# irap-omp/deconv3d

Hardware: AMD Instinct MI355X
Metric: spaxel-updates/sec (MH-Gibbs) (higher is better)
Workload: dtype f64; 1 GPU; c3_300x300x128; fsf=moffat 11x11, lsf_taps=17, spaxels=90000, lsf=analytic MUSE stand-in (mpdaf absent), parallelism=1 chain, variance=per-voxel cube (heteroscedastic)

## Files before the change

deconv3d_amd/csrc/d3d_api.hip:

```cpp
#include "d3d_ctx.h"

#include <dlfcn.h>

#define D3D_VERSION 300
#ifndef D3D_SOURCE_HASH
#define D3D_SOURCE_HASH "unknown"
#endif

namespace {
thread_local std::string g_err;
}

namespace d3dh {
int fail(int code, const char *fmt, ...) {
    char buf[512];
    va_list ap;
    va_start(ap, fmt);
    vsnprintf(buf, sizeof buf, fmt, ap);
    va_end(ap);
    g_err = buf;
    return code;
}
}

// ... 89 lines not shown
    c->mh_nt_ivar = c->mh_nt_ivar && fits_raw;
    c->mh_layers_forced = c->mh_layers_opt > 0;
    c->mh_layers_cfg = c->mh_layers_forced ? c->mh_layers_opt : 2;
    if (c->mh_layers_cfg < 1) c->mh_layers_cfg = 1;
    if (c->mh_layers_cfg > d3d::MH_LAYERS) c->mh_layers_cfg = d3d::MH_LAYERS;
    if (c->Dp > 160 && c->mh_layers_cfg > 2) c->mh_layers_cfg = 2;
    c->mh_defer = c->mh_defer_opt;
    c->mh_zb = c->mh_zblocks && c->Dp > d3d::MH_WS_MAX_DP && c->mh_defer == 1 && !c->mh_flow &&
               (!c->have_taps || c->ntaps == 0 || c->lsf_dense_any);
    if (c->mh_defer != 1 || c->mh_flow || (c->Dp > d3d::MH_WS_MAX_DP && !c->mh_zb)) c->mh_layers_cfg = 1;
    if (c->deep && !c->mh_zb) c->mh_defer = 0;
    c->mh_layers = c->mh_layers_cfg;
}

int floor_div(int a, int b) { return a >= 0 ? a / b : -((-a + b - 1) / b); }

int build_colour_lists(d3d_ctx *c) {
    const int ncol = c->fh * c->fw;
    const int fhh = (c->fh - 1) / 2, fhw = (c->fw - 1) / 2;
    c->parts.clear();
    if (c->part_rects.empty()) {
        d3d_ctx::Part pt;
        pt.y0 = c->oy0;
        pt.y1 = c->oy1;
        pt.x0 = c->ox0;
        pt.x1 = c->ox1;
        c->parts.push_back(pt);
        c->n_phases = 1;
    } else {
        c->n_phases = 1;
// ... 45 lines not shown
                    }
                if (pt.real[col] > 0) {
                    const long n_all_col =
                        ((long)list.size() - pt.off[col]) * (c->mh_zb ? (c->Dp + 255) / 256 : 1);
                    if (c->mh_zigzag && (ord & 1) && n_all_col > c->flow_grid) {
                        std::reverse(list.begin() + pt.off[col], list.begin() + pt.off[col] + pt.real[col]);
                        std::reverse(list.begin() + pt.off[col] + pt.real[col], list.end());
                    }
                    ++ord;
                }
                most = std::max(most, (int)list.size() - pt.off[col]);
            }
        pt.off[ncol] = (int)list.size();
        const long most_wgs = (long)most * (c->mh_zb ? (c->Dp + 255) / 256 : 1);
        pt.layers = (!c->mh_layers_forced && most_wgs < c->flow_grid / 2) ? 1 : c->mh_layers_cfg;
        const bool partitioned = c->tiled || !c->part_rects.empty();
        pt.wide = pt.layers == 1 && c->mh_wide && partitioned && c->Dp == 128 && most > 0 &&
                  most <= c->flow_grid / 4 && c->mh_defer == 1;
        pt.small = pt.layers == 1 && most_wgs < c->flow_grid / 2;
        pt.chain = false;
        pt.K = 0;
        pt.last_col = -1;
        for (int col = 0; col < ncol; ++col)
            if (pt.real[col] > 0) {
                ++pt.K;
                pt.last_col = col;
            }
#ifdef D3D_EXPERIMENTS
        if (!empty && pt.K > 0) {
            const int cus = c->flow_grid / 4;
// ... 50 lines not shown
                HIP_TRY(hipMemsetAsync(c->chain_flags, 0, 2 * need_slots * sizeof(unsigned), c->stream));
                c->chain_base = 0;
            }
            if (need_G > c->chain_G_cap) {
                if (c->chain_G) (void)hipFree(c->chain_G);
                c->chain_G = nullptr;
                c->chain_G_cap = 0;
                HIP_TRY(hipMalloc(&c->chain_G, need_G * sizeof(double)));
                c->chain_G_cap = need_G;
            }
            HIP_TRY(hipStreamSynchronize(c->stream));
        }
    }
    c->mh_layers = 1;
    for (const d3d_ctx::Part &pt : c->parts) c->mh_layers = std::max(c->mh_layers, pt.layers);
    if (list.size() > c->spx_cap) {
        if (c->spx) (void)hipFree(c->spx);
        c->spx = nullptr;
        c->spx_cap = 0;
        HIP_TRY(hipMalloc(&c->spx, list.size() * sizeof(int4)));
        c->spx_cap = list.size();
    }
    c->flow_K = 0;
    c->flow_items = 0;
    c->flow_last_cy = c->flow_last_cx = -1;
#ifdef D3D_EXPERIMENTS
    if (!c->tiled && c->parts.size() == 1 && list.size() <= c->flow_cap_items) {
        const d3d_ctx::Part &pt = c->parts[0];
        std::vector<int4> ents, cols;
        std::vector<int> lat((size_t)ncol * c->flow_LY * c->flow_LX, -1);
// ... 314 lines not shown
    CTX_TRY(hipMalloc(&c->dlog, (size_t)c->HW * sizeof(double)));
    CTX_TRY(hipMalloc(&c->hwbuf, (size_t)c->HW * sizeof(double)));
    CTX_TRY(hipMalloc(&c->scal, 16 * sizeof(double)));
    CTX_TRY(hipMalloc(&c->accepted, sizeof(unsigned long long)));
    CTX_TRY(hipMalloc(&c->acc_map, (size_t)c->HW * sizeof(unsigned)));
    c->spx_cap = (size_t)(H + 2 * fh) * (W + 2 * fw);
    CTX_TRY(hipMalloc(&c->spx, c->spx_cap * sizeof(int4)));
    c->slots_x = (W + fw - 1) / fw;
    c->slots = c->slots_x * ((H + fh - 1) / fh);
    c->Wg = W;
    c->oy1 = H;
    c->ox1 = W;
    CTX_TRY(hipMalloc(&c->prev, (size_t)c->HW * 3 * sizeof(double)));
    CTX_TRY(hipMalloc(&c->recbuf, (size_t)c->HW * 8 * sizeof(double)));
    CTX_TRY(hipMalloc(&c->idxbuf, (size_t)c->HW * sizeof(int)));
    for (int b = 0; b < 4; ++b) {
        CTX_TRY(hipMalloc(&c->gbuf[b], (size_t)c->slots * c->Dp * sizeof(double)));
        CTX_TRY(hipMemsetAsync(c->gbuf[b], 0, (size_t)c->slots * c->Dp * sizeof(double), c->stream));
    }
    {
#ifdef D3D_EXPERIMENTS
        const size_t ncol = (size_t)fh * fw;
        c->flow_LY = H / fh + 3;
        c->flow_LX = W / fw + 3;
        c->flow_cap_K = ncol;
        c->flow_cap_items = c->spx_cap;
        CTX_TRY(hipMalloc(&c->flow_ent, c->spx_cap * sizeof(int4)));
        CTX_TRY(hipMalloc(&c->flow_col, ncol * sizeof(int4)));
        CTX_TRY(hipMalloc(&c->flow_lat, ncol * c->flow_LY * c->flow_LX * sizeof(int)));
        c->flow_state_bytes = ((4 + ncol + c->spx_cap) * sizeof(unsigned) + 15) / 16 * 16;
        CTX_TRY(hipMalloc(&c->flow_state, c->flow_state_bytes));
// ... 32 lines not shown
    }
    if (c->copy_stream) (void)hipStreamDestroy(c->copy_stream);
    if (c->halo_send) (void)hipFree(c->halo_send);
    if (c->halo_recv) (void)hipFree(c->halo_recv);
    for (double *p : c->post_cube)
        if (p) (void)hipFree(p);
    if (c->post_map) (void)hipFree(c->post_map);
    hist_free(c);
    adapt_free(c);
    if (c->prior_part) (void)hipFree(c->prior_part);
    for (hipEvent_t e : c->halo_ev) (void)hipEventDestroy(e);
    for (int s = 0; s < D3D_SLOT_COUNT; ++s)
        if (c->slot[s]) (void)hipFree(c->slot[s]);
    if (c->line.tab) (void)hipFree(const_cast<double *>(c->line.tab));
    void *ptrs[] = {c->stage, c->stage2, c->params, c->params_alt, c->mask, c->fsf, c->lsf_shift, c->lsf_weight,
                    c->dlog, c->hwbuf, c->scal, c->accepted, c->acc_map, c->spx, c->gbuf[0], c->gbuf[1], c->gbuf[2], c->gbuf[3],
                    c->flow_ent, c->flow_col, c->flow_lat, c->flow_state, c->flow_err, c->pair_state, c->sep_uv,
                    c->lsf_dense, c->prev, c->recbuf, c->idxbuf, c->extbuf, c->fsf_quad, c->fsf_quad_sep,
                    c->chain_cols, c->chain_flags, c->chain_G, c->props, c->z_part, c->z_E, c->ltab, c->ptab};
    for (void *p : ptrs)
        if (p) (void)hipFree(p);
#ifdef D3D_EXPERIMENTS
    if (c->stampbuf) (void)hipFree(c->stampbuf);
#endif
    if (c->ev0) (void)hipEventDestroy(c->ev0);
    if (c->ev1) (void)hipEventDestroy(c->ev1);
    if (c->own_stream) (void)hipStreamDestroy(c->own_stream);
    delete c;
    return D3D_OK;
}

// ... 73 lines not shown
        long n = 0;
        for (const d3d_ctx::Part &pt : c->parts) n += pt.chain ? 1 : 0;
        *value = c->have_data ? n : 0;
        return D3D_OK;
    }
    if (!strcmp(key, "search_bank_ns") || !strcmp(key, "search_kernel_ns")) {
        *value = key[7] == 'b' ? c->search_bank_ns : c->search_kernel_ns;
        return D3D_OK;
    }
    if (!strcmp(key, "prep_median_ns") || !strcmp(key, "prep_stats_ns")) {
        *value = key[5] == 'm' ? c->prep_median_ns : c->prep_stats_ns;
        return D3D_OK;
    }
    if (!strcmp(key, "mh_nt_ivar_on")) {
        *value = c->mh_nt_ivar ? 1 : 0;
        return D3D_OK;
    }
    if (!strcmp(key, "batch_layers")) {
        *value = c->batch_layers;
        return D3D_OK;
    }
    if (!strcmp(key, "lsf_fits")) {
        *value = (c->have_taps && (c->ntaps == 0 || c->lsf_dense_any)) ? 1 : 0;
        return D3D_OK;
    }
    if (!strcmp(key, "lsf_taps")) {
        *value = c->ntaps;
        return D3D_OK;
    }
    if (!strcmp(key, "spatial_path") || !strcmp(key, "spectral_path") || !strcmp(key, "stage_path")) {
// ... 1510 lines not shown
```

deconv3d_amd/csrc/d3d_ctx.h:

```cpp
#pragma once
#include <hip/hip_runtime.h>
#include <rccl/rccl.h>

#include <algorithm>
#include <cmath>
#include <cstdarg>
#include <cstdio>
#include <cstdlib>
#include <cstring>
#include <new>
#include <string>
#include <vector>

#include "../../include/deconv3d_hip.h"
#include "d3d_kernels.h"

#ifndef D3D_WIDE_NS
#define D3D_WIDE_NS 704
#endif
constexpr int MH_WIDE_NS = D3D_WIDE_NS;
constexpr int MH_CHAIN_NT = 768;

namespace d3dh {
int fail(int code, const char *fmt, ...);
// ... 98 lines not shown
    int mh_nt_opt = 0, mh_maxit_opt = -1;
    int mh_defer = 1;
    int mh_defer_opt = 1;
    int mh_zblocks = 1;
    bool mh_zb = false;
    double *z_part = nullptr;
    double *z_E = nullptr;
    size_t z_part_cap = 0;
#ifdef D3D_EXPERIMENTS
    unsigned long long *stampbuf = nullptr;
    size_t stamp_launches = 0, stamp_next = 0, stamp_stride = 0;
#endif
    bool ivar_is_uniform = false;
    double ivar_uniform = 0.0;
    int uniform_fast_path = 1;
    double *gbuf[4] = {nullptr, nullptr, nullptr, nullptr};
    int lay_n = 0, lay_cy[3] = {-1, -1, -1}, lay_cx[3] = {-1, -1, -1}, lay_g[3] = {0, 0, 0};
    int mh_layers = 2;
    int batch_layers = 0;
    bool mh_nt_ivar = false;
    int mh_nt_ivar_opt = -1;
    int mh_zigzag = 1;
    int mh_layers_opt = 0;
    int mh_layers_cfg = 2;
    bool mh_layers_forced = false;
    int mh_flow = 0;
    int flow_K = 0, flow_LY = 0, flow_LX = 0, flow_items = 0, flow_grid = 0;
    int flow_last_cy = -1, flow_last_cx = -1;
    int mh_chain_opt = 0;
    int2 *chain_cols = nullptr;
    size_t chain_cols_cap = 0;
    unsigned *chain_flags = nullptr;
    size_t chain_slots_cap = 0;
    double *chain_G = nullptr;
    size_t chain_G_cap = 0;
    unsigned chain_base = 0;
    bool chain_used = false;
    int mh_props = 1;
    d3d::MHProposal *props = nullptr;
    long props_sweep = -1;
// ... 123 lines not shown
int halo_exchange(d3d_ctx *c, int plan);

void colour_residue(const d3d_ctx *c, int col, int *cy, int *cx);

void pend_clear(d3d_ctx *c);
int pend_free_buf(const d3d_ctx *c);
void pend_push(d3d_ctx *c, int cy, int cx, int g);
void fill_mh_args(d3d_ctx *c, d3d::MHArgs &P);
int launch_mh(d3d_ctx *c, const d3d::MHArgs &P, unsigned grid, uint32_t sweep);
int launch_mh_zb(d3d_ctx *c, d3d::MHArgs &P, unsigned n_items, uint32_t sweep, int layers);
int launch_mh_batch(d3d_ctx *c, const d3d::MHArgs &P, unsigned grid, uint32_t sweep, int layers);
void fill_chain_args(const d3d_ctx *c, d3d::MHChainArgs &B, bool tables);
int launch_mh_defer(d3d_ctx *c, const d3d::MHArgs &P, unsigned grid, uint32_t sweep, int layers,
                    bool wide);
int flush_pending(d3d_ctx *c);
int ensure_proposals(d3d_ctx *c, uint32_t sweep);
int ensure_tables(d3d_ctx *c, bool lines);
int ensure_ptab(d3d_ctx *c);
int launch_line_table(d3d_ctx *c, const d3d::MHArgs &P, uint32_t sweep, const d3d::MHChainArgs *chains, int R);
bool mh_small_usable(const d3d_ctx *c);
int mh_ptab_row(const d3d_ctx *c, int ly, int lx, int layer = 0);
bool mh_part_uses_tables(const d3d_ctx *c, const d3d_ctx::Part &pt);
#ifdef D3D_EXPERIMENTS
int launch_mh_chain(d3d_ctx *c, int pi, uint32_t sweep0, int n_sweeps);
#endif
int launch_apply_updates(d3d_ctx *c, const d3d::MHArgs &P, const double *rec, int n);
int launch_rtnorm(d3d_ctx *c, long n, double lo, double hi, double mu, double sigma, uint64_t seed,
                  int wave_mode, double *buf);
int launch_philox(d3d_ctx *c, long n, const uint32_t *counters, const uint32_t *keys, uint32_t *words,
                  double *pairs);
// ... 9 lines not shown
```

deconv3d_amd/csrc/d3d_kernels.h:

```cpp
#pragma once
#include <hip/hip_runtime.h>
#include <stdint.h>

#include "d3d_rng.h"

namespace d3d {


static __global__ __launch_bounds__(256) void k_to_device_layout(const double *__restrict__ src,
                                                           double *__restrict__ dst, int D,
                                                           int Dp, long HW) {
    __shared__ double tile[32][33];
    const int tx = threadIdx.x & 31, ty = threadIdx.x >> 5;
    const long s0 = (long)blockIdx.x * 32;
    const int z0 = blockIdx.y * 32;
#pragma unroll
    for (int k = 0; k < 32; k += 8) {
        const int z = z0 + ty + k;
        const long s = s0 + tx;
        tile[ty + k][tx] = (z < D && s < HW) ? src[(long)z * HW + s] : 0.0;
    }
    __syncthreads();
#pragma unroll
    for (int k = 0; k < 32; k += 8) {
// ... 1439 lines not shown
                                               double *__restrict__ out) {
    __shared__ double part[16];
    double acc = 0.0;
    for (long i = threadIdx.x; i < n; i += 1024) acc += v[i];
    acc = wave_sum(acc);
    if ((threadIdx.x & 63) == 0) part[threadIdx.x >> 6] = acc;
    __syncthreads();
    if (threadIdx.x == 0) {
        double t = 0.0;
        for (int i = 0; i < 16; ++i) t += part[i];
        *out = t;
    }
}


struct MHProposal;
struct MHChainArgs {
    double *err;
    const double *ivar;
    double ivar_uniform;
    double *params, *prev, *dlog;
    unsigned long long *accepted;
    double *gbuf[4];
    double min_b[3], max_b[3], amp[3];
    double ra;
    uint64_t seed;
    const MHProposal *props;
    const double *ltab;
    const double *jscale;
    unsigned *jacc;
    double lam[3];
    int prior;
    unsigned *acc_map;
};
struct MHArgs {
    int D, Dp, HL, H, W, fh, fw, N, ntaps, npos;
    double *err;
    const double *ivar;
// ... 4 lines not shown
    const int *shift;
    const double *weight;
    double *dlog;
    unsigned long long *accepted;
    const int4 *spx;
    double min_b[3], max_b[3], amp[3];
    double ra;
    uint64_t seed;
    int gy0, gx0, Wg;
    int dy0, dy1, dx0, dx1;
    const uint8_t *mask;
    const double *Gprev;
    double *Gcur;
    int n_lay, write_back;
    int rev;
    int lay_cy[3], lay_cx[3];
    const double *lay_G[3];
    int prev_cy, prev_cx;
    int slots_x;
    const int *ext_idx;
    const double *ext_in;
    const double *ext_lines;
    double *ext_out;
    int ext_gibbs;
    int probe;
    int probe_sp;
    double probe_p[3];
    double *probe_out;
    const MHProposal *props;
    double *z_part;
    double *z_E;
    int z_nb, z_db, z_slots;
    const struct MHChainArgs *batch;
    int b_items, b_gcur, b_lay_g[3];
    int prio;
    const double *ltab;
    int fw_inv;
    const double *ptab;
    int ptab_row[2];
    LineShape line;
#ifdef D3D_EXPERIMENTS
    unsigned long long *stamp;
#endif
    const double *jscale;
    unsigned *jacc;
    double lam[3];
    int prior;
    unsigned *acc_map;
};

#ifdef D3D_EXPERIMENTS
#define D3D_MH_STAMP(at, k, who)                                                      \
    do {                                                                              \
        if (P.stamp && threadIdx.x == (who)) P.stamp[(long)(at) * 8 + (k)] = wall_clock64(); \
    } while (0)
#else
#define D3D_MH_STAMP(at, k, who)
#endif

constexpr int MH_LAYERS = 3;
constexpr int MH_WS_MAX_DP = 512;

__device__ __forceinline__ void mh_stagger(int prio) {
    prio &= 63;
    if (prio <= 0) return;
    if (prio < 16) {
        if ((blockIdx.x >> (prio - 1)) & 1) __builtin_amdgcn_s_setprio(2);
    } else if (blockIdx.x & 1) {
        for (int i = 16; i < prio; ++i) __builtin_amdgcn_s_sleep(30);
    }
}

__host__ __device__ inline size_t mh_lds_doubles(int NT, int HL, int Dp, int N, int npos,
                                                 int M = 1) {
    const int G = NT / HL;
// ... 765 lines not shown
                const int j = ch + LSF_RL + (sh > Z.Nfull / 2 ? sh - Z.Nfull : sh);
                const double wt = P.weight[t];
                eo = fma(wt, LO[j], eo);
                en = fma(wt, LN[j], en);
            }
        } else {
            eo = LO[ch + LSF_RL];
            en = LN[ch + LSF_RL];
        }
    }
    *EO = eo;
    *EN = en;
}

template <int NS, bool UV, bool COH, int U, int M, bool COHG = COH, bool PRE = false, bool NTV = false,
          bool PROPS = false, bool ZBK = false, bool MULTI = false, bool PRIOR = false>
__device__ __forceinline__ void mh_ws_run(const MHArgs &P, const MHShared &S, const MHWsItem &I,
                                          uint32_t sweep, long stamp_at,
                                          const MHPre<U> *pre = nullptr, const MHZ *Zp = nullptr,
                                          int item = 0, int zb = 0) {
    const long zstride = ZBK ? Zp->zs : (long)P.Dp;
    constexpr int ROW = 1 + M;
    const int tid = threadIdx.x;
    const int HL = P.HL, Dp = P.Dp, N = P.N;
    const int G = NS / HL;
    double *sEN = S.sum + 8 * (NS / 64) + 8;
    MHProposal *sq = reinterpret_cast<MHProposal *>(sEN + Dp);
    MHPrior *spt = reinterpret_cast<MHPrior *>(sq + 1);
    static_assert(sizeof(MHProposal) + sizeof(MHPrior) <= 16 * sizeof(double), "LDS behind the lines");
    const bool real = I.real != 0;
    const int sp = I.y * P.W + I.x;
// ... 7 lines not shown
        if (g < G) {
            double2 sA = make_double2(0.0, 0.0), sB = sA, sC = sA;
            const double2 vu = make_double2(P.ivar_uniform,
                                            (2 * zl + 1 < P.D) ? P.ivar_uniform : 0.0);
            typedef unsigned v4u __attribute__((ext_vector_type(4)));
            union { double2 d; v4u i; } cv;
            long rs_vox = 0;
            if constexpr (NTV && !COH) {
                const int fhh_ = (P.fh - 1) / 2, fhw_ = (P.fw - 1) / 2;
                rs_vox = max(0L, (long)(I.y - fhh_) * P.W + (I.x - fhw_));
            }
            const long rs_bytes =
                (COH || NTV) ? ((long)P.H * P.W - rs_vox) * zstride * 8 - (ZBK ? Zp->z0 : 0) * 8 : 0;
            const __amdgpu_buffer_rsrc_t err_rsrc = __builtin_amdgcn_make_buffer_rsrc(
                P.err + rs_vox * zstride, 0, (int)(unsigned)min(rs_bytes, 0x7fffffffL), 0x00020000);
            auto issue = [&](int p0, int (&vox)[U], double2 (&e)[U], double2 (&v)[U]) {
#pragma unroll
                for (int u = 0; u < U; ++u) {
                    const int pw = p0 + u * G;
                    const int p = I.rev ? P.npos - 1 - pw : pw;
                    vox[u] = (pw < P.npos) ? S.pos[ROW * p] : -1;
                    const long idx = (long)max(vox[u], 0) * zstride + 2 * zl;
                    if (COH) {
                        cv.i = __builtin_amdgcn_raw_buffer_load_b128(err_rsrc, (int)(idx * 8), 0, 16);
                        e[u] = cv.d;
                    } else {
                        e[u] = *reinterpret_cast<const double2 *>(P.err + idx);
                    }
                    v[u] = vu;
#ifdef D3D_EXPERIMENTS
                    if (!UV && !(P.prio & 128)) v[u] = mh_load_ivar<NTV>(P.ivar + idx);
#else
                    if (!UV) v[u] = mh_load_ivar<NTV>(P.ivar + idx);
#endif
                }
            };
            auto consume = [&](int p0, int (&vox)[U], double2 (&e)[U], double2 (&v)[U]) {
#pragma unroll
                for (int u = 0; u < U; ++u) {
                    if (vox[u] < 0) continue;
                    const int pw = p0 + u * G;
                    const int p = I.rev ? P.npos - 1 - pw : pw;
                    const long idx = (long)vox[u] * zstride + 2 * zl;
                    bool touched = false;
#pragma unroll
                    for (int j = 0; j < M; ++j) {
                        const int code = (j < I.n_lay) ? S.pos[ROW * p + 1 + j] : -1;
                        if (code >= 0) {
                            const double fp = S.fsf[code & 0xffff];
                            const double2 gz = *reinterpret_cast<const double2 *>(
                                S.gp + ((size_t)j * 4 + (code >> 16)) * Dp + 2 * zl);
                            e[u].x = fma(fp, gz.x, e[u].x);
                            e[u].y = fma(fp, gz.y, e[u].y);
                            touched = true;
                        }
                    }
#ifdef D3D_EXPERIMENTS
                    if (P.prio & 64) touched = false;
#endif
                    if (touched && I.write_back) {
                        if (COH || NTV) {
                            cv.d = e[u];
                            __builtin_amdgcn_raw_buffer_store_b128(
                                cv.i, err_rsrc, (int)((idx - rs_vox * zstride) * 8), 0, 16);
                        } else {
                            *reinterpret_cast<double2 *>(P.err + idx) = e[u];
                        }
                    }
                    const double f = S.fsf[p];
                    D3D_ACCUM(e[u], v[u], f);
                }
            };
            int p0 = g;
            if constexpr (PRE) {
                int vox[U];
                double2 e[U], v[U];
#pragma unroll
                for (int u = 0; u < U; ++u) {
                    vox[u] = pre->vox[u];
                    e[u] = pre->e[u];
                    v[u] = UV ? vu : pre->v[u];
                }
                consume(p0, vox, e, v);
                p0 += U * G;
            }
            constexpr int UNR = U >= 8 ? 1 : 4;
#pragma unroll UNR
            for (; p0 < P.npos; p0 += U * G) {
                int vox[U];
                double2 e[U], v[U];
                issue(p0, vox, e, v);
                consume(p0, vox, e, v);
            }
            if (real) {
                double *r = S.red + (size_t)g * 3 * Dp + 2 * zl;
                r[0] = sA.x;
                r[1] = sA.y;
                r[Dp] = sB.x;
                r[Dp + 1] = sB.y;
                r[2 * Dp] = sC.x;
                r[2 * Dp + 1] = sC.y;
            }
        }
    } else if (real) {
        const int lane = tid - NS;
        const MHProposal q = PROPS ? mh_proposal_of(P, sp, sweep) : mh_propose(P, sp, sweep);
        if constexpr (ZBK) {
// ... 152 lines not shown
    D3D_MH_STAMP(blockIdx.x, 0, 0);
#ifdef D3D_EXPERIMENTS
    if (P.stamp && threadIdx.x == 0)
        P.stamp[(long)blockIdx.x * 8 + 5] =
            (unsigned long long)__builtin_amdgcn_s_getreg(4 | (0 << 6) | (31 << 11)) |
            ((unsigned long long)__builtin_amdgcn_s_getreg(20 | (0 << 6) | (3 << 11)) << 32);
    mh_stagger(P.prio);
#endif
    const int4 ent = P.spx[BATCH ? item : (int)blockIdx.x];
    MHWsItem I;
    I.y = ent.x;
    I.x = ent.y;
    I.real = ent.z;
    mh_ws_layers_from_args(P, I);
    if constexpr (NL >= 0) I.n_lay = NL;
    if (!I.real && (I.n_lay == 0 || !I.write_back)) {
        mh_ws_zero_row<false>(P, I);
        return;
    }
    mh_ws_preds<M>(P, I);
    MHGpRegs<M, K> gv;
    mh_ws_gp_load<M, K, false>(P, I, NT, gv);
    const double tap0 = ((int)threadIdx.x < P.npos) ? P.fsf[threadIdx.x] : 0.0;
    MHPre<U> pre;
    mh_ws_prefetch<NS, UV, U, NTV>(P, I, pre);
    mh_ws_table<M>(P, S, I, NT, &tap0);
    mh_ws_gp_store<M, K>(P, S, I, NT, gv);
    __syncthreads();
    D3D_MH_STAMP(blockIdx.x, 1, 0);
    mh_ws_run<NS, UV, false, U, M, false, true, NTV, (U >= 4 || NS != 256), false, MULTI, PRIOR>(P, S, I, sweep, blockIdx.x,
                                                                           &pre);
}

#ifdef D3D_EXPERIMENTS
struct MHChain {
    const int2 *cols;
    unsigned *flag1;
    unsigned *flag2;
    unsigned *err;
    double *G;
    double *Gout;
    int K, n_sy, n_sx;
    int sy0, sx0;
    int py0, py1, px0, px1;
    unsigned base;
    uint32_t sweep0;
// ... 1136 lines not shown
```

deconv3d_amd/csrc/d3d_mh.hip:

```cpp
#include "d3d_ctx.h"
#include "d3d_mh_small.h"

namespace d3dh {

using namespace d3d;

void pend_clear(d3d_ctx *c) {
    c->lay_n = 0;
    c->pend_part = -1;
}

int pend_free_buf(const d3d_ctx *c) {
    for (int b = 0; b < 4; ++b) {
        bool used = false;
        for (int j = 0; j < c->lay_n; ++j) used = used || c->lay_g[j] == b;
        if (!used) return b;
    }
    return 0;
}

void pend_push(d3d_ctx *c, int cy, int cx, int g) {
    c->lay_cy[c->lay_n] = cy;
    c->lay_cx[c->lay_n] = cx;
    c->lay_g[c->lay_n] = g;
    ++c->lay_n;
}

template <class A>
// ... 9 lines not shown
    for (int k = 0; k < 3; ++k) {
        a.min_b[k] = c->min_b[k];
        a.max_b[k] = c->max_b[k];
        a.amp[k] = c->amp[k];
        a.lam[k] = c->prior_on ? c->prior_lam[k] : 0.0;
    }
    a.ra = c->ra;
    a.seed = c->seed;
    a.jscale = c->adapt_on ? c->jscale : nullptr;
    a.jacc = c->adapt_on ? c->jacc : nullptr;
    a.prior = c->prior_on ? 1 : 0;
}

void fill_chain_args(const d3d_ctx *c, d3d::MHChainArgs &B, bool tables) {
    fill_chain_fields(c, B);
    for (int b = 0; b < 4; ++b) B.gbuf[b] = c->gbuf[b];
    B.props = tables ? c->props : nullptr;
    B.ltab = tables ? c->ltab : nullptr;
}

void fill_mh_args(d3d_ctx *c, d3d::MHArgs &P) {
    fill_chain_fields(c, P);
    P.D = c->D;
    P.Dp = c->Dp;
    P.HL = c->HL;
    P.H = c->H;
    P.W = c->W;
    P.fh = c->fh;
    P.fw = c->fw;
    P.N = c->N;
    P.ntaps = c->ntaps;
// ... 1 lines not shown
    P.fsf = c->fsf;
    P.shift = c->lsf_shift;
    P.weight = c->lsf_weight;
    P.spx = c->spx;
    P.rev = 0;
    P.prio = c->mh_prio;
    P.props = nullptr;
    P.ltab = nullptr;
    P.fw_inv = (65536 + c->fw - 1) / c->fw;
    P.ptab = nullptr;
    P.ptab_row[0] = P.ptab_row[1] = c->fh * c->fw;
    P.line = c->line;
    P.batch = nullptr;
    P.b_items = 0;
    P.b_gcur = 0;
    P.b_lay_g[0] = P.b_lay_g[1] = P.b_lay_g[2] = 0;
    P.z_part = c->z_part;
    P.z_E = c->z_E;
    P.z_db = 256;
    P.z_nb = (c->Dp + P.z_db - 1) / P.z_db;
    P.z_slots = (int)c->slots;
    P.gy0 = c->gy0;
    P.gx0 = c->gx0;
    P.Wg = c->Wg;
    if (c->pend_part >= 0 && c->pend_part < (int)c->parts.size()) {
        const d3d_ctx::Part &pt = c->parts[c->pend_part];
        P.dy0 = pt.dy0;
        P.dy1 = pt.dy1;
        P.dx0 = pt.dx0;
        P.dx1 = pt.dx1;
    } else {
        P.dy0 = 0;
        P.dy1 = c->H;
        P.dx0 = 0;
        P.dx1 = c->W;
    }
    P.mask = c->mask;
    P.n_lay = c->lay_n;
    P.write_back = 1;
    for (int j = 0; j < 3; ++j) {
        const bool live = j < c->lay_n;
        P.lay_cy[j] = live ? c->lay_cy[j] : -1;
        P.lay_cx[j] = live ? c->lay_cx[j] : -1;
        P.lay_G[j] = c->gbuf[live ? c->lay_g[j] : 0];
    }
    P.Gcur = c->gbuf[pend_free_buf(c)];
    const int last = c->lay_n - 1;
    P.Gprev = c->gbuf[last >= 0 ? c->lay_g[last] : 0];
    P.prev_cy = last >= 0 ? c->lay_cy[last] : -1;
    P.prev_cx = last >= 0 ? c->lay_cx[last] : -1;
    P.slots_x = c->slots_x;
    P.ext_idx = nullptr;
    P.ext_in = nullptr;
    P.ext_lines = nullptr;
    P.ext_out = nullptr;
// ... 130 lines not shown
}

template <int NT>
int launch_mh_defer_nt(d3d_ctx *c, const d3d::MHArgs &P, unsigned grid, uint32_t sweep) {
    const size_t lds = d3d::mh_lds_doubles(NT, c->HL, c->Dp, c->N, P.npos) * sizeof(double);
    auto kern = P.prior ? (d3d::line_multi(c->line) ? &d3d::k_mh_defer<NT, true, true> : &d3d::k_mh_defer<NT, false, true>)
                        : (d3d::line_multi(c->line) ? &d3d::k_mh_defer<NT, true> : &d3d::k_mh_defer<NT, false>);
    hipLaunchKernelGGL(kern, dim3(grid), dim3(NT), lds, c->stream, P, sweep);
    HIP_TRY(hipGetLastError());
    return 0;
}

template <bool UV, int U, int M, int K, bool NTV = false, int NS = 256>
int launch_mh_ws_um(d3d_ctx *c, const d3d::MHArgs &P, unsigned grid, uint32_t sweep) {
    const size_t lds = d3d::mh_ws_lds_doubles(NS, c->HL, c->Dp, c->N, P.npos, M) * sizeof(double);
    hipError_t attr = hipSuccess;
    auto go = [&](auto kern) {
        if (lds > 65536)
            attr = hipFuncSetAttribute(reinterpret_cast<const void *>(kern),
                                       hipFuncAttributeMaxDynamicSharedMemorySize, (int)lds);
        hipLaunchKernelGGL(kern, dim3(grid), dim3(NS + 64), lds, c->stream, P, sweep);
    };
    switch (P.n_lay <= M ? P.n_lay : -1) {
        case 0: go(mh_ws_kernel<NS, UV, U, M, K, 0, NTV>(d3d::line_multi(P.line), P.prior != 0)); break;
        case 1: go(mh_ws_kernel<NS, UV, U, M, K, 1, NTV>(d3d::line_multi(P.line), P.prior != 0)); break;
        case 2:
            if constexpr (M >= 2) go(mh_ws_kernel<NS, UV, U, M, K, 2, NTV>(d3d::line_multi(P.line), P.prior != 0));
            break;
        case 3:
            if constexpr (M >= 3) go(mh_ws_kernel<NS, UV, U, M, K, 3, NTV>(d3d::line_multi(P.line), P.prior != 0));
            break;
        default:
            return fail(D3D_ERR_STATE, "internal: %d pending layers for a %d-layer kernel", P.n_lay, M);
    }
    HIP_TRY(attr);
    HIP_TRY(hipGetLastError());
    return 0;
}

bool mh_small_usable(const d3d_ctx *c) {
    return c->mh_small && c->mh_props && c->mh_defer == 1 && !c->mh_zb && !c->deep && c->Dp <= 256 &&
           c->fh <= 31 && c->fw <= 31 && (double)c->cube_elems * 8.0 < 4294967296.0;
}

int mh_ptab_row(const d3d_ctx *c, int ly, int lx, int layer) {
// ... 107 lines not shown
        if constexpr (!UV) ntv = c->mh_nt_ivar && !(grid < (unsigned)c->flow_grid / 2);
        const bool few = grid < (unsigned)c->flow_grid / 2;
        if (layers >= 2) {
            if (few) return launch_mh_ws_um<UV, 4, 2, 4, false, 512>(c, P, grid, sweep);
            if constexpr (!UV)
                if (ntv) return launch_mh_ws_um<UV, 4, 2, 4, true, 512>(c, P, grid, sweep);
            return launch_mh_ws_um<UV, 4, 2, 4, false, 512>(c, P, grid, sweep);
        }
        if (few) return launch_mh_ws_um<UV, 4, 1, 4, false, 512>(c, P, grid, sweep);
        if constexpr (!UV)
            if (ntv) return launch_mh_ws_um<UV, 1, 1, 4, true, 512>(c, P, grid, sweep);
        return launch_mh_ws_um<UV, 1, 1, 4, false, 512>(c, P, grid, sweep);
    }
    if constexpr (!UV) {
        if (c->mh_nt_ivar && !small) {
            if (layers >= 3) return launch_mh_ws_um<UV, 2, 3, 2, true>(c, P, grid, sweep);
            if (layers == 2) {
                if (c->Dp > 160) return launch_mh_ws_um<UV, 2, 2, 4, true>(c, P, grid, sweep);
                return launch_mh_ws_um<UV, 2, 2, 2, true>(c, P, grid, sweep);
            }
            return launch_mh_ws_um<UV, 1, 1, 4, true>(c, P, grid, sweep);
        }
    }
    if (layers >= 3) {
        if (small) return launch_mh_ws_um<UV, 4, 3, 2>(c, P, grid, sweep);
        return launch_mh_ws_um<UV, 2, 3, 2>(c, P, grid, sweep);
    }
    if (layers == 2) {
        if (c->Dp > 160) {
            if (small) return launch_mh_ws_um<UV, 4, 2, 4>(c, P, grid, sweep);
            return launch_mh_ws_um<UV, 2, 2, 4>(c, P, grid, sweep);
        }
        if (small) return launch_mh_ws_um<UV, 4, 2, 2>(c, P, grid, sweep);
        return launch_mh_ws_um<UV, 2, 2, 2>(c, P, grid, sweep);
    }
    if (small && wide) return launch_mh_ws_um<UV, 1, 1, 1, false, MH_WIDE_NS>(c, P, grid, sweep);
    if (small) return launch_mh_ws_um<UV, 4, 1, 4>(c, P, grid, sweep);
    return launch_mh_ws_um<UV, 1, 1, 4>(c, P, grid, sweep);
}
// ... 186 lines not shown
            if (nl == 0) go(mh_ws_kernel<NS, UV, 2, 2, 2, 0, false, false, true>(d3d::line_multi(P.line), P.prior != 0), 2);
            else if (nl == 1) go(mh_ws_kernel<NS, UV, 2, 2, 2, 1, false, false, true>(d3d::line_multi(P.line), P.prior != 0), 2);
            else go(mh_ws_kernel<NS, UV, 2, 2, 2, 2, false, false, true>(d3d::line_multi(P.line), P.prior != 0), 2);
        }
    } else {
        if (nl == 0) go(mh_ws_kernel<NS, UV, 4, 1, 4, 0, false, false, true>(d3d::line_multi(P.line), P.prior != 0), 1);
        else go(mh_ws_kernel<NS, UV, 4, 1, 4, 1, false, false, true>(d3d::line_multi(P.line), P.prior != 0), 1);
    }
    HIP_TRY(hipGetLastError());
    return 0;
}

int launch_mh_batch(d3d_ctx *c, const d3d::MHArgs &P, unsigned grid, uint32_t sweep, int layers) {
    if (c->ivar_is_uniform && c->uniform_fast_path) return launch_mh_batch_t<true>(c, P, grid, sweep, layers);
    return launch_mh_batch_t<false>(c, P, grid, sweep, layers);
}

int launch_mh_defer(d3d_ctx *c, const d3d::MHArgs &P, unsigned grid, uint32_t sweep, int layers,
                    bool wide) {
    if (c->mh_defer == 1 && c->Dp <= d3d::MH_WS_MAX_DP) {
        if (c->ivar_is_uniform && c->uniform_fast_path)
            return launch_mh_ws<true>(c, P, grid, sweep, layers, wide);
        return launch_mh_ws<false>(c, P, grid, sweep, layers, wide);
    }
    switch (c->mh_nt) {
        case 128: return launch_mh_defer_nt<128>(c, P, grid, sweep);
        case 256: return launch_mh_defer_nt<256>(c, P, grid, sweep);
        case 512: return launch_mh_defer_nt<512>(c, P, grid, sweep);
        default: return launch_mh_defer_nt<1024>(c, P, grid, sweep);
    }
// ... 199 lines not shown
```

deconv3d_amd/csrc/d3d_sweep.hip:

```cpp
#include "d3d_ctx.h"

using namespace d3dh;

void d3dh::colour_residue(const d3d_ctx *c, int col, int *cy, int *cx) {
    *cy = ((col / c->fw - c->gy0) % c->fh + c->fh) % c->fh;
    *cx = ((col % c->fw - c->gx0) % c->fw + c->fw) % c->fw;
}

namespace {

struct SnapQueue {
    int slot[d3d_ctx::STREAM_NB];
    int head = 0, count = 0;
};

int snap_setup(d3d_ctx *c) {
    if (c->copy_stream) return 0;
    HIP_TRY(hipStreamCreateWithFlags(&c->copy_stream, hipStreamNonBlocking));
    const size_t bytes = (size_t)c->HW * 4 * sizeof(double);
    for (int b = 0; b < d3d_ctx::STREAM_NB; ++b) {
        HIP_TRY(hipMalloc(&c->snap_dev[b], bytes));
        HIP_TRY(hipHostMalloc((void **)&c->snap_host[b], bytes, hipHostMallocDefault));
        HIP_TRY(hipEventCreateWithFlags(&c->snap_ready[b], hipEventDisableTiming));
        HIP_TRY(hipEventCreateWithFlags(&c->snap_done[b], hipEventDisableTiming));
// ... 132 lines not shown
        if (!deferred) {
            if (int rc = launch_mh(c, P, (unsigned)n_real, sweep)) return rc;
            continue;
        }
        const int n_all = pt.off[col + 1] - pt.off[col];
#ifdef D3D_EXPERIMENTS
        if (!b && c->stampbuf && c->stamp_next < c->stamp_launches && (size_t)n_all * 8 <= c->stamp_stride)
            P.stamp = c->stampbuf + (c->stamp_next++) * c->stamp_stride;
#endif
        const int g_cur = pend_free_buf(c);
        int rc;
        if (b) {
            P.batch = b->dev;
            P.b_items = n_all;
            P.b_gcur = g_cur;
            for (int j = 0; j < 3; ++j) P.b_lay_g[j] = j < c->lay_n ? c->lay_g[j] : 0;
            rc = launch_mh_batch(c, P, (unsigned)n_all * b->R, sweep, layers);
        } else {
            rc = c->mh_zb ? launch_mh_zb(c, P, (unsigned)n_all, sweep, layers)
                          : launch_mh_defer(c, P, (unsigned)n_all, sweep, layers, pt.wide);
        }
        if (rc) return rc;
        for (int r = 0; r < (b ? b->R : 1); ++r) push_colour_layer(cs[r], pi, col, g_cur, P.write_back);
    }
    return 0;
}

int run_phase(d3d_ctx *c, int phase, uint32_t sweep) {
    for (size_t pi = 0; pi < c->parts.size(); ++pi)
        if (c->parts[pi].phase == phase)
            if (int rc = run_part(c, (int)pi, sweep)) return rc;
// ... 277 lines not shown
```

Before: 18.59 million spaxel-updates/s.

## Support four deferred MH layers, prefetch layer operands, and specialise write-back

```diff
diff --git a/deconv3d_amd/csrc/d3d_api.hip b/deconv3d_amd/csrc/d3d_api.hip
--- a/deconv3d_amd/csrc/d3d_api.hip
+++ b/deconv3d_amd/csrc/d3d_api.hip
@@ -127,6 +127,9 @@
 }
 
 int floor_div(int a, int b) { return a >= 0 ? a / b : -((-a + b - 1) / b); }
+
+constexpr int MH_AUTO_LAYERS_GENERAL = 2;
+constexpr int MH_AUTO_LAYERS_UNIFORM = 2;
 
 int build_colour_lists(d3d_ctx *c) {
     const int ncol = c->fh * c->fw;
@@ -202,6 +205,17 @@
         pt.off[ncol] = (int)list.size();
         const long most_wgs = (long)most * (c->mh_zb ? (c->Dp + 255) / 256 : 1);
         pt.layers = (!c->mh_layers_forced && most_wgs < c->flow_grid / 2) ? 1 : c->mh_layers_cfg;
+        if (!c->mh_layers_forced && pt.layers == 2 && c->Dp > 64 && c->Dp <= 160) {
+            const bool uv = c->ivar_is_uniform && c->uniform_fast_path;
+            for (int d = uv ? MH_AUTO_LAYERS_UNIFORM : MH_AUTO_LAYERS_GENERAL; d > 2; --d) {
+                long resident = 0;
+                if (int rc = d3dh::mh_ws_resident(c, d, &resident)) return rc;
+                if (most_wgs <= resident) {
+                    pt.layers = d;
+                    break;
+                }
+            }
+        }
         const bool partitioned = c->tiled || !c->part_rects.empty();
         pt.wide = pt.layers == 1 && c->mh_wide && partitioned && c->Dp == 128 && most > 0 &&
                   most <= c->flow_grid / 4 && c->mh_defer == 1;
@@ -282,6 +296,7 @@
     }
     c->mh_layers = 1;
     for (const d3d_ctx::Part &pt : c->parts) c->mh_layers = std::max(c->mh_layers, pt.layers);
+    if (int rc = d3dh::mh_ws_resident(c, c->mh_layers, &c->mh_resident)) return rc;
     if (list.size() > c->spx_cap) {
         if (c->spx) (void)hipFree(c->spx);
         c->spx = nullptr;
@@ -626,7 +641,7 @@
     CTX_TRY(hipMalloc(&c->prev, (size_t)c->HW * 3 * sizeof(double)));
     CTX_TRY(hipMalloc(&c->recbuf, (size_t)c->HW * 8 * sizeof(double)));
     CTX_TRY(hipMalloc(&c->idxbuf, (size_t)c->HW * sizeof(int)));
-    for (int b = 0; b < 4; ++b) {
+    for (int b = 0; b <= d3d::MH_LAYERS; ++b) {
         CTX_TRY(hipMalloc(&c->gbuf[b], (size_t)c->slots * c->Dp * sizeof(double)));
         CTX_TRY(hipMemsetAsync(c->gbuf[b], 0, (size_t)c->slots * c->Dp * sizeof(double), c->stream));
     }
@@ -689,7 +704,7 @@
         if (c->slot[s]) (void)hipFree(c->slot[s]);
     if (c->line.tab) (void)hipFree(const_cast<double *>(c->line.tab));
     void *ptrs[] = {c->stage, c->stage2, c->params, c->params_alt, c->mask, c->fsf, c->lsf_shift, c->lsf_weight,
-                    c->dlog, c->hwbuf, c->scal, c->accepted, c->acc_map, c->spx, c->gbuf[0], c->gbuf[1], c->gbuf[2], c->gbuf[3],
+                    c->dlog, c->hwbuf, c->scal, c->accepted, c->acc_map, c->spx, c->gbuf[0], c->gbuf[1], c->gbuf[2], c->gbuf[3], c->gbuf[4],
                     c->flow_ent, c->flow_col, c->flow_lat, c->flow_state, c->flow_err, c->pair_state, c->sep_uv,
                     c->lsf_dense, c->prev, c->recbuf, c->idxbuf, c->extbuf, c->fsf_quad, c->fsf_quad_sep,
                     c->chain_cols, c->chain_flags, c->chain_G, c->props, c->z_part, c->z_E, c->ltab, c->ptab};
@@ -793,6 +808,10 @@
     }
     if (!strcmp(key, "mh_nt_ivar_on")) {
         *value = c->mh_nt_ivar ? 1 : 0;
+        return D3D_OK;
+    }
+    if (!strcmp(key, "mh_resident")) {
+        *value = c->have_data ? c->mh_resident : 0;
         return D3D_OK;
     }
     if (!strcmp(key, "batch_layers")) {
diff --git a/deconv3d_amd/csrc/d3d_ctx.h b/deconv3d_amd/csrc/d3d_ctx.h
--- a/deconv3d_amd/csrc/d3d_ctx.h
+++ b/deconv3d_amd/csrc/d3d_ctx.h
@@ -136,8 +136,9 @@
     bool ivar_is_uniform = false;
     double ivar_uniform = 0.0;
     int uniform_fast_path = 1;
-    double *gbuf[4] = {nullptr, nullptr, nullptr, nullptr};
-    int lay_n = 0, lay_cy[3] = {-1, -1, -1}, lay_cx[3] = {-1, -1, -1}, lay_g[3] = {0, 0, 0};
+    double *gbuf[d3d::MH_LAYERS + 1] = {};
+    int lay_n = 0, lay_cy[d3d::MH_LAYERS] = {-1, -1, -1, -1}, lay_cx[d3d::MH_LAYERS] = {-1, -1, -1, -1},
+        lay_g[d3d::MH_LAYERS] = {0, 0, 0, 0};
     int mh_layers = 2;
     int batch_layers = 0;
     bool mh_nt_ivar = false;
@@ -146,6 +147,7 @@
     int mh_layers_opt = 0;
     int mh_layers_cfg = 2;
     bool mh_layers_forced = false;
+    long mh_resident = 0;
     int mh_flow = 0;
     int flow_K = 0, flow_LY = 0, flow_LX = 0, flow_items = 0, flow_grid = 0;
     int flow_last_cy = -1, flow_last_cx = -1;
@@ -299,6 +301,7 @@
 int launch_mh_defer(d3d_ctx *c, const d3d::MHArgs &P, unsigned grid, uint32_t sweep, int layers,
                     bool wide);
 int flush_pending(d3d_ctx *c);
+int mh_ws_resident(d3d_ctx *c, int layers, long *out);
 int ensure_proposals(d3d_ctx *c, uint32_t sweep);
 int ensure_tables(d3d_ctx *c, bool lines);
 int ensure_ptab(d3d_ctx *c);
diff --git a/deconv3d_amd/csrc/d3d_kernels.h b/deconv3d_amd/csrc/d3d_kernels.h
--- a/deconv3d_amd/csrc/d3d_kernels.h
+++ b/deconv3d_amd/csrc/d3d_kernels.h
@@ -1477,6 +1477,8 @@
 }
 
 
+constexpr int MH_LAYERS = 4;
+
 struct MHProposal;
 struct MHChainArgs {
     double *err;
@@ -1484,7 +1486,7 @@
     double ivar_uniform;
     double *params, *prev, *dlog;
     unsigned long long *accepted;
-    double *gbuf[4];
+    double *gbuf[MH_LAYERS + 1];
     double min_b[3], max_b[3], amp[3];
     double ra;
     uint64_t seed;
@@ -1519,8 +1521,8 @@
     double *Gcur;
     int n_lay, write_back;
     int rev;
-    int lay_cy[3], lay_cx[3];
-    const double *lay_G[3];
+    int lay_cy[MH_LAYERS], lay_cx[MH_LAYERS];
+    const double *lay_G[MH_LAYERS];
     int prev_cy, prev_cx;
     int slots_x;
     const int *ext_idx;
@@ -1537,7 +1539,7 @@
     double *z_E;
     int z_nb, z_db, z_slots;
     const struct MHChainArgs *batch;
-    int b_items, b_gcur, b_lay_g[3];
+    int b_items, b_gcur, b_lay_g[MH_LAYERS];
     int prio;
     const double *ltab;
     int fw_inv;
@@ -1563,7 +1565,6 @@
 #define D3D_MH_STAMP(at, k, who)
 #endif
 
-constexpr int MH_LAYERS = 3;
 constexpr int MH_WS_MAX_DP = 512;
 
 __device__ __forceinline__ void mh_stagger(int prio) {
@@ -2359,7 +2360,7 @@
 }
 
 template <int NS, bool UV, bool COH, int U, int M, bool COHG = COH, bool PRE = false, bool NTV = false,
-          bool PROPS = false, bool ZBK = false, bool MULTI = false, bool PRIOR = false>
+          bool PROPS = false, bool ZBK = false, bool MULTI = false, bool PRIOR = false, int WB = -1>
 __device__ __forceinline__ void mh_ws_run(const MHArgs &P, const MHShared &S, const MHWsItem &I,
                                           uint32_t sweep, long stamp_at,
                                           const MHPre<U> *pre = nullptr, const MHZ *Zp = nullptr,
@@ -2397,7 +2398,38 @@
                 (COH || NTV) ? ((long)P.H * P.W - rs_vox) * zstride * 8 - (ZBK ? Zp->z0 : 0) * 8 : 0;
             const __amdgpu_buffer_rsrc_t err_rsrc = __builtin_amdgcn_make_buffer_rsrc(
                 P.err + rs_vox * zstride, 0, (int)(unsigned)min(rs_bytes, 0x7fffffffL), 0x00020000);
-            auto issue = [&](int p0, int (&vox)[U], double2 (&e)[U], double2 (&v)[U]) {
+            struct LayOps {
+                int code[U][M];
+                double fp[U][M], f[U];
+                double2 gz[U][M];
+            };
+            constexpr bool LEAN = M >= 3;
+            constexpr int PF = (LEAN || U * M > 6) ? 1 : U;
+            constexpr bool GZA = !LEAN;
+            auto operands = [&](int p0, int u, LayOps &L) {
+                const int pw = p0 + u * G;
+                const int p = (pw < P.npos) ? (I.rev ? P.npos - 1 - pw : pw) : 0;
+#pragma unroll
+                for (int j = 0; j < M; ++j) {
+                    L.code[u][j] = -1;
+                    if (j < I.n_lay) {
+                        const int c = S.pos[ROW * p + 1 + j];
+                        L.code[u][j] = (pw < P.npos) ? c : -1;
+                    }
+                }
+                L.f[u] = S.fsf[p];
+#pragma unroll
+                for (int j = 0; j < M; ++j) {
+                    if (j < I.n_lay) {
+                        const int c = max(L.code[u][j], 0);
+                        L.fp[u][j] = S.fsf[c & 0xffff];
+                        if constexpr (GZA)
+                            L.gz[u][j] = *reinterpret_cast<const double2 *>(
+                                S.gp + ((size_t)j * 4 + (c >> 16)) * Dp + 2 * zl);
+                    }
+                }
+            };
+            auto issue = [&](int p0, int (&vox)[U], double2 (&e)[U], double2 (&v)[U], LayOps &L) {
 #pragma unroll
                 for (int u = 0; u < U; ++u) {
                     const int pw = p0 + u * G;
@@ -2417,31 +2449,34 @@
                     if (!UV) v[u] = mh_load_ivar<NTV>(P.ivar + idx);
 #endif
                 }
+#pragma unroll
+                for (int u = 0; u < PF; ++u) operands(p0, u, L);
             };
-            auto consume = [&](int p0, int (&vox)[U], double2 (&e)[U], double2 (&v)[U]) {
+            auto consume = [&](int p0, int (&vox)[U], double2 (&e)[U], double2 (&v)[U], LayOps &L) {
 #pragma unroll
                 for (int u = 0; u < U; ++u) {
+                    if constexpr (PF < U) {
+                        __builtin_amdgcn_sched_barrier(0);
+                        if (u + PF < U) operands(p0, u + PF, L);
+                    }
                     if (vox[u] < 0) continue;
-                    const int pw = p0 + u * G;
-                    const int p = I.rev ? P.npos - 1 - pw : pw;
                     const long idx = (long)vox[u] * zstride + 2 * zl;
                     bool touched = false;
 #pragma unroll
                     for (int j = 0; j < M; ++j) {
-                        const int code = (j < I.n_lay) ? S.pos[ROW * p + 1 + j] : -1;
-                        if (code >= 0) {
-                            const double fp = S.fsf[code & 0xffff];
-                            const double2 gz = *reinterpret_cast<const double2 *>(
-                                S.gp + ((size_t)j * 4 + (code >> 16)) * Dp + 2 * zl);
-                            e[u].x = fma(fp, gz.x, e[u].x);
-                            e[u].y = fma(fp, gz.y, e[u].y);
+                        if (j < I.n_lay && L.code[u][j] >= 0) {
+                            if constexpr (!GZA)
+                                L.gz[u][j] = *reinterpret_cast<const double2 *>(
+                                    S.gp + ((size_t)j * 4 + (L.code[u][j] >> 16)) * Dp + 2 * zl);
+                            e[u].x = fma(L.fp[u][j], L.gz[u][j].x, e[u].x);
+                            e[u].y = fma(L.fp[u][j], L.gz[u][j].y, e[u].y);
                             touched = true;
                         }
                     }
 #ifdef D3D_EXPERIMENTS
                     if (P.prio & 64) touched = false;
 #endif
-                    if (touched && I.write_back) {
+                    if (touched && (WB >= 0 ? WB != 0 : I.write_back != 0)) {
                         if (COH || NTV) {
                             cv.d = e[u];
                             __builtin_amdgcn_raw_buffer_store_b128(
@@ -2450,21 +2485,23 @@
                             *reinterpret_cast<double2 *>(P.err + idx) = e[u];
                         }
                     }
-                    const double f = S.fsf[p];
-                    D3D_ACCUM(e[u], v[u], f);
+                    D3D_ACCUM(e[u], v[u], L.f[u]);
                 }
             };
             int p0 = g;
             if constexpr (PRE) {
                 int vox[U];
                 double2 e[U], v[U];
+                LayOps L;
 #pragma unroll
                 for (int u = 0; u < U; ++u) {
                     vox[u] = pre->vox[u];
                     e[u] = pre->e[u];
                     v[u] = UV ? vu : pre->v[u];
                 }
-                consume(p0, vox, e, v);
+#pragma unroll
+                for (int u = 0; u < PF; ++u) operands(p0, u, L);
+                consume(p0, vox, e, v, L);
                 p0 += U * G;
             }
             constexpr int UNR = U >= 8 ? 1 : 4;
@@ -2472,8 +2509,9 @@
             for (; p0 < P.npos; p0 += U * G) {
                 int vox[U];
                 double2 e[U], v[U];
-                issue(p0, vox, e, v);
-                consume(p0, vox, e, v);
+                LayOps L;
+                issue(p0, vox, e, v, L);
+                consume(p0, vox, e, v, L);
             }
             if (real) {
                 double *r = S.red + (size_t)g * 3 * Dp + 2 * zl;
@@ -2656,6 +2694,8 @@
     I.real = ent.z;
     mh_ws_layers_from_args(P, I);
     if constexpr (NL >= 0) I.n_lay = NL;
+    constexpr int WB = (NL >= 0 && !BATCH) ? (NL == M ? 1 : 0) : -1;
+    if constexpr (WB >= 0) I.write_back = WB;
     if (!I.real && (I.n_lay == 0 || !I.write_back)) {
         mh_ws_zero_row<false>(P, I);
         return;
@@ -2670,8 +2710,8 @@
     mh_ws_gp_store<M, K>(P, S, I, NT, gv);
     __syncthreads();
     D3D_MH_STAMP(blockIdx.x, 1, 0);
-    mh_ws_run<NS, UV, false, U, M, false, true, NTV, (U >= 4 || NS != 256), false, MULTI, PRIOR>(P, S, I, sweep, blockIdx.x,
-                                                                           &pre);
+    mh_ws_run<NS, UV, false, U, M, false, true, NTV, (U >= 4 || NS != 256), false, MULTI, PRIOR, WB>(P, S, I, sweep, blockIdx.x,
+                                                                               &pre);
 }
 
 #ifdef D3D_EXPERIMENTS
diff --git a/deconv3d_amd/csrc/d3d_mh.hip b/deconv3d_amd/csrc/d3d_mh.hip
--- a/deconv3d_amd/csrc/d3d_mh.hip
+++ b/deconv3d_amd/csrc/d3d_mh.hip
@@ -11,7 +11,7 @@
 }
 
 int pend_free_buf(const d3d_ctx *c) {
-    for (int b = 0; b < 4; ++b) {
+    for (int b = 0; b <= d3d::MH_LAYERS; ++b) {
         bool used = false;
         for (int j = 0; j < c->lay_n; ++j) used = used || c->lay_g[j] == b;
         if (!used) return b;
@@ -51,7 +51,7 @@
 
 void fill_chain_args(const d3d_ctx *c, d3d::MHChainArgs &B, bool tables) {
     fill_chain_fields(c, B);
-    for (int b = 0; b < 4; ++b) B.gbuf[b] = c->gbuf[b];
+    for (int b = 0; b <= d3d::MH_LAYERS; ++b) B.gbuf[b] = c->gbuf[b];
     B.props = tables ? c->props : nullptr;
     B.ltab = tables ? c->ltab : nullptr;
 }
@@ -83,7 +83,7 @@
     P.batch = nullptr;
     P.b_items = 0;
     P.b_gcur = 0;
-    P.b_lay_g[0] = P.b_lay_g[1] = P.b_lay_g[2] = 0;
+    for (int j = 0; j < d3d::MH_LAYERS; ++j) P.b_lay_g[j] = 0;
     P.z_part = c->z_part;
     P.z_E = c->z_E;
     P.z_db = 256;
@@ -107,7 +107,7 @@
     P.mask = c->mask;
     P.n_lay = c->lay_n;
     P.write_back = 1;
-    for (int j = 0; j < 3; ++j) {
+    for (int j = 0; j < d3d::MH_LAYERS; ++j) {
         const bool live = j < c->lay_n;
         P.lay_cy[j] = live ? c->lay_cy[j] : -1;
         P.lay_cx[j] = live ? c->lay_cx[j] : -1;
@@ -268,6 +268,8 @@
 template <bool UV, int U, int M, int K, bool NTV = false, int NS = 256>
 int launch_mh_ws_um(d3d_ctx *c, const d3d::MHArgs &P, unsigned grid, uint32_t sweep) {
     const size_t lds = d3d::mh_ws_lds_doubles(NS, c->HL, c->Dp, c->N, P.npos, M) * sizeof(double);
+    NEED((P.write_back != 0) == (P.n_lay == M) || P.n_lay == 0, D3D_ERR_STATE,
+         "internal: write_back %d with %d pending layers of %d", P.write_back, P.n_lay, M);
     hipError_t attr = hipSuccess;
     auto go = [&](auto kern) {
         if (lds > 65536)
@@ -283,6 +285,9 @@
             break;
         case 3:
             if constexpr (M >= 3) go(mh_ws_kernel<NS, UV, U, M, K, 3, NTV>(d3d::line_multi(P.line), P.prior != 0));
+            break;
+        case 4:
+            if constexpr (M >= 4) go(mh_ws_kernel<NS, UV, U, M, K, 4, NTV>(d3d::line_multi(P.line), P.prior != 0));
             break;
         default:
             return fail(D3D_ERR_STATE, "internal: %d pending layers for a %d-layer kernel", P.n_lay, M);
@@ -420,7 +425,8 @@
     }
     if constexpr (!UV) {
         if (c->mh_nt_ivar && !small) {
-            if (layers >= 3) return launch_mh_ws_um<UV, 2, 3, 2, true>(c, P, grid, sweep);
+            if (layers >= 4) return launch_mh_ws_um<UV, 2, 4, 2, true>(c, P, grid, sweep);
+            if (layers == 3) return launch_mh_ws_um<UV, 2, 3, 2, true>(c, P, grid, sweep);
             if (layers == 2) {
                 if (c->Dp > 160) return launch_mh_ws_um<UV, 2, 2, 4, true>(c, P, grid, sweep);
                 return launch_mh_ws_um<UV, 2, 2, 2, true>(c, P, grid, sweep);
@@ -428,7 +434,11 @@
             return launch_mh_ws_um<UV, 1, 1, 4, true>(c, P, grid, sweep);
         }
     }
-    if (layers >= 3) {
+    if (layers >= 4) {
+        if (small) return launch_mh_ws_um<UV, 4, 4, 2>(c, P, grid, sweep);
+        return launch_mh_ws_um<UV, 2, 4, 2>(c, P, grid, sweep);
+    }
+    if (layers == 3) {
         if (small) return launch_mh_ws_um<UV, 4, 3, 2>(c, P, grid, sweep);
         return launch_mh_ws_um<UV, 2, 3, 2>(c, P, grid, sweep);
     }
@@ -645,6 +655,30 @@
 int launch_mh_batch(d3d_ctx *c, const d3d::MHArgs &P, unsigned grid, uint32_t sweep, int layers) {
     if (c->ivar_is_uniform && c->uniform_fast_path) return launch_mh_batch_t<true>(c, P, grid, sweep, layers);
     return launch_mh_batch_t<false>(c, P, grid, sweep, layers);
+}
+
+template <bool UV, int M, int K>
+static int mh_ws_resident_t(d3d_ctx *c, int *per_cu) {
+    constexpr int NS = 256;
+    const size_t lds = d3d::mh_ws_lds_doubles(NS, c->HL, c->Dp, c->N, c->fh * c->fw, M) * sizeof(double);
+    auto kern = mh_ws_kernel<NS, UV, (UV ? 4 : 2), M, K, M>(d3d::line_multi(c->line), c->prior_on);
+    HIP_TRY(hipOccupancyMaxActiveBlocksPerMultiprocessor(per_cu, reinterpret_cast<const void *>(kern), NS + 64,
+                                                         lds));
+    return 0;
+}
+
+int mh_ws_resident(d3d_ctx *c, int layers, long *out) {
+    *out = 0;
+    if (c->mh_defer != 1 || c->mh_zb || c->Dp > 256 || layers < 2 || (layers > 2 && c->Dp > 160)) return 0;
+    const bool uv = c->ivar_is_uniform && c->uniform_fast_path;
+    int per_cu = 0, rc;
+    if (layers >= 4) rc = uv ? mh_ws_resident_t<true, 4, 2>(c, &per_cu) : mh_ws_resident_t<false, 4, 2>(c, &per_cu);
+    else if (layers == 3) rc = uv ? mh_ws_resident_t<true, 3, 2>(c, &per_cu) : mh_ws_resident_t<false, 3, 2>(c, &per_cu);
+    else if (c->Dp > 160) rc = uv ? mh_ws_resident_t<true, 2, 4>(c, &per_cu) : mh_ws_resident_t<false, 2, 4>(c, &per_cu);
+    else rc = uv ? mh_ws_resident_t<true, 2, 2>(c, &per_cu) : mh_ws_resident_t<false, 2, 2>(c, &per_cu);
+    if (rc) return rc;
+    *out = (long)per_cu * (c->flow_grid / 4);
+    return 0;
 }
 
 int launch_mh_defer(d3d_ctx *c, const d3d::MHArgs &P, unsigned grid, uint32_t sweep, int layers,
diff --git a/deconv3d_amd/csrc/d3d_sweep.hip b/deconv3d_amd/csrc/d3d_sweep.hip
--- a/deconv3d_amd/csrc/d3d_sweep.hip
+++ b/deconv3d_amd/csrc/d3d_sweep.hip
@@ -170,7 +170,7 @@
             P.batch = b->dev;
             P.b_items = n_all;
             P.b_gcur = g_cur;
-            for (int j = 0; j < 3; ++j) P.b_lay_g[j] = j < c->lay_n ? c->lay_g[j] : 0;
+            for (int j = 0; j < d3d::MH_LAYERS; ++j) P.b_lay_g[j] = j < c->lay_n ? c->lay_g[j] : 0;
             rc = launch_mh_batch(c, P, (unsigned)n_all * b->R, sweep, layers);
         } else {
             rc = c->mh_zb ? launch_mh_zb(c, P, (unsigned)n_all, sweep, layers)
```

Measured after the change: 18.67 million spaxel-updates/s, median of 6. No clear change (+0.4%).
